# mstebelev/wormhole

Hardware: AMD Instinct MI355X
Metric: examples/sec, DiFacto FM on Criteo-1TB-shaped sparse at 1/2/4/8 MI355X (higher is better)
Workload: dtype fp32; 1 GPU; model=difacto-fm-dim64, global_batch=100000, seq_len=39, parallelism=dp1+kvshard1, minibatch_per_gpu=100000, threshold=100, nnz_per_example=39

## Files before the change

### csrc/bind/fm_ops.cc

```cpp
#include "kv_store.h"
#include "localize_ahead.h"
#include "ps_ops.h"
#include "step_rt.h"
#include "store_guard.h"

#include <c10/hip/HIPCachingAllocator.h>
#include <c10/hip/HIPGuard.h>

#include <cmath>
#include <cstring>
#include <memory>

#include "host/linear_guard_plan.h"

namespace wh_bind {
namespace {

void check_vstride(int64_t vstride) {
  TORCH_CHECK(vstride == 0 || (vstride >= 4 && vstride <= 256 && (vstride & (vstride - 1)) == 0),
              "vstride must be 0 or 4 * 2^k <= 256, got ", vstride);
}

int loss_flags(int64_t loss, const Tensor& met) {
  return (int)loss | (met.numel() >= 5 ? 256 : 0);
// ... 554 lines not shown
      const bool fuse_now = fused_v_ && vc.data_ptr() == store_->V_.data_ptr();
      auto bw = fm_backward_impl(csc_off, csc_row, csc_val, fw[1], fw[2], hdr, vc, vs_,
                                 fuse_now ? &fuse : nullptr, planned ? &bwd : nullptr);
      if (post_on_)
        fm_grad_post(bw[1], m, dim_, clip_, dropout_, seed_ + 7919 * step + 1, gnorm_);
      ht.mark(4);
      auc_acc_side(fw[0], label, auc_sum);
      ht.mark(6);
      store_->difacto_push_after(slot, hdr, bw[0], bw[1], hp_, threshold_, l1_shrk_, seed_,
                                 fuse_now ? c10::optional<Tensor>(ucnt) : c10::nullopt);
      ht.mark(5);
    } else if (train) {
      auc_acc_side(fw[0], label, auc_sum);
    }
    return py::make_tuple(fw[0], U, m);
  }

  void reset() { ahead_.reset(); }
  bool direct() const { return direct_; }
  bool fused_v() const { return fused_v_; }
  int64_t grows() const { return guard_.grows(); }
  int64_t vgrows() const { return guard_.vgrows(); }
  std::vector<int64_t> guard_sync() {
    if (guard_.stale()) guard_.after();
    return guard_.sync();
  }

 private:
  KVStore* store_;
  std::vector<double> hp_;
  int64_t threshold_;
  bool l1_shrk_;
  int64_t seed_, loss_;
  int vs_ = 0;
  double clip_ = 0, dropout_ = 0;
  bool gnorm_ = false, post_on_ = false, direct_ = false, fused_v_ = false;
  int64_t dim_ = 0;
  StoreGuard guard_;
  LocalizeAhead ahead_;
  std::unique_ptr<HostSplit> timing_{host_split("difacto native step")};
};

}

void bind_fm(py::module_& m) {
  py::class_<LinearStep>(m, "LinearStep")
      .def(py::init<KVStore*, int64_t, double, double, double, double, int64_t, double, bool>(),
           py::arg("store"), py::arg("algo"), py::arg("alpha"), py::arg("beta"), py::arg("l1"),
           py::arg("l2"), py::arg("loss"), py::arg("max_load") = 0.7, py::arg("direct") = true,
           py::keep_alive<1, 2>())
      .def("step", &LinearStep::step, py::arg("keys"), py::arg("offset"), py::arg("val"),
           py::arg("label"), py::arg("train"), py::arg("met"), py::arg("auc_sum"),
           py::arg("next_keys") = py::none(), py::arg("next_offset") = py::none(),
           py::arg("next_val") = py::none(), py::arg("ready") = 0)
      .def("reset", &LinearStep::reset)
      .def("guard_sync", &LinearStep::guard_sync)
      .def_property_readonly("grows", &LinearStep::grows)
      .def_property_readonly("direct", [](const LinearStep& l) { return l.direct(); })
      .def_property("pushes", &LinearStep::pushes, &LinearStep::set_pushes);
  py::class_<DifactoStep>(m, "DifactoStep")
      .def(py::init<KVStore*, std::vector<double>, int64_t, bool, int64_t, int64_t,
                    std::vector<double>, double, bool, bool>(),
           py::arg("store"), py::arg("hp"), py::arg("threshold"), py::arg("l1_shrk"),
           py::arg("seed"), py::arg("loss"), py::arg("post"), py::arg("max_load"),
           py::arg("direct"), py::arg("fused_v") = true, py::keep_alive<1, 2>())
      .def("step", &DifactoStep::step, py::arg("keys"), py::arg("offset"), py::arg("val"),
           py::arg("label"), py::arg("train"), py::arg("data_pass"), py::arg("met"),
           py::arg("auc_sum"), py::arg("step"), py::arg("next_keys") = py::none(),
           py::arg("next_offset") = py::none(), py::arg("next_val") = py::none(),
           py::arg("ready") = 0)
      .def("reset", &DifactoStep::reset)
      .def("guard_sync", &DifactoStep::guard_sync)
      .def_property_readonly("direct", &DifactoStep::direct)
      .def_property_readonly("fused_v", &DifactoStep::fused_v)
      .def_property_readonly("grows", &DifactoStep::grows)
      .def_property_readonly("vgrows", &DifactoStep::vgrows);
  m.def("fm_forward", &fm_forward);
  m.def("set_cu_reserve", [](int64_t n) { wh::fm_set_cu_reserve((int)n); },
        "CUs the persistent FM kernels leave free for concurrent collectives");
  m.def("cu_reserve", []() { return (int64_t)wh::fm_cu_reserve(); });
  m.def("set_fm_bwd_pack", [](bool on) { wh::fm_set_bwd_pack(on); },
        "FM backward: pack small single-chunk keys, one lane group per key (default on)");
  m.def("fm_bwd_pack", []() { return wh::fm_bwd_pack(); });
  m.def("fm_backward", &fm_backward);
  m.def("fm_backward_plan", &fm_backward_plan, py::arg("csc_off"), py::arg("csc_row"),
        py::arg("hdr"), py::arg("vc_rows"), py::arg("nrows"), py::arg("vstride"),
        py::arg("two_pass") = false);
  m.def("fm_backward_run", &fm_backward_run);
  m.def("difacto_open_pull_plan", &difacto_open_pull_plan, py::arg("store"), py::arg("keys"),
        py::arg("insert"), py::arg("cnt"), py::arg("h"), py::arg("threshold"),
        py::arg("l1_shrk"), py::arg("seed"), py::arg("direct"), py::arg("csc_off"),
        py::arg("csc_row"), py::arg("nrows"),
        "(tests) the open with the backward's chunk plan: (slot, hdr, vc, vpos, plan)");
  m.def("fm_backward_plan_totals", &fm_backward_plan_totals, py::arg("plan"),
        py::arg("csc_off"), py::arg("nnz"), py::arg("vstride"),
        "(tests) a backward plan's chunk totals {scalar, V}");
  m.def("fm_grad_post", &fm_grad_post);
  m.def("vstride_for", &vstride_for);
  m.def("spmv_t", &spmv_t, py::arg("csc_off"), py::arg("csc_row"), py::arg("csc_val"),
        py::arg("p"));
}

}
```

### csrc/hip/fm.hip

```cpp
#include "wh_common.h"
#include <string>
#include "kv_device.h"
#include "wh_chunk_plan.h"
#include "wh_kernels.h"
#include "wh_lookback.h"
#include "wh_loss.h"

#include <algorithm>
#include <cstdlib>
#include <type_traits>

namespace wh {
namespace {

constexpr int kThreads = 256;
constexpr int kFwdBlocks = 2048;

template <int G>
struct Shape {
  static constexpr int SUB = 64 / G;
  static constexpr int NI = G;
#ifndef WH_FM_TI
#define WH_FM_TI 4
#endif
  static constexpr int TI = G < WH_FM_TI ? G : WH_FM_TI;
  static constexpr int VS = 4 * G;
};

__device__ float kZeroRow[256];

template <int G>
__device__ __forceinline__ void stage_pairs(int2* st, int lane, int idx_val, float f) {
  using S = Shape<G>;
  st[(lane % S::SUB) * S::NI + lane / S::SUB] = make_int2(idx_val, __float_as_int(f));
  __builtin_amdgcn_fence(__ATOMIC_RELEASE, "wavefront");
  __builtin_amdgcn_wave_barrier();
  __builtin_amdgcn_fence(__ATOMIC_ACQUIRE, "wavefront");
}

template <int G>
__device__ __forceinline__ int stage_pairs_compact(int2* st, int lane, int vid, float f) {
  using S = Shape<G>;
  const bool has = vid >= 0;
  const uint64_t m = __ballot(has);
  const int nv = __popcll(m);
  const int pos = __popcll(m & ((1ull << lane) - 1ull));
  if (has) st[(pos % S::SUB) * S::NI + pos / S::SUB] = make_int2(vid, __float_as_int(f));
  __builtin_amdgcn_fence(__ATOMIC_RELEASE, "wavefront");
  __builtin_amdgcn_wave_barrier();
  __builtin_amdgcn_fence(__ATOMIC_ACQUIRE, "wavefront");
  return nv;
}

template <int G>
__global__ __launch_bounds__(kThreads) void k_fm_fwd(int64_t nrows, const int64_t* __restrict__ off,
                                                     const int32_t* __restrict__ lid,
                                                     const float* __restrict__ val,
                                                     const float2* __restrict__ hdr,
                                                     const float* __restrict__ vc, int vstride,
                                                     const float* __restrict__ label, int loss,
                                                     float* __restrict__ py_out,
                                                     float* __restrict__ dual_out,
                                                     float* __restrict__ xv, double* part,
                                                     double* met, unsigned int* ticket, int acc5) {
  using S = Shape<G>;
  __shared__ double sh[kThreads / 64];
  __shared__ int2 stage[kThreads / 64][64];
  const int lane = threadIdx.x & 63, gl = lane & (G - 1), sub = lane / G;
  const int64_t nw = (int64_t)gridDim.x * (kThreads / 64);
  const int64_t w0 =
      __builtin_amdgcn_readfirstlane((int)(((int64_t)blockIdx.x * kThreads + threadIdx.x) >> 6));
  double m_objv = 0, m_objw = 0, m_corr = 0, m_n = 0;
  auto bounds = [&](int64_t r, int64_t& b, int64_t& e) {
    if (r < nrows) {
      b = off[r];
      e = off[r + 1];
    } else {
      b = e = 0;
    }
  };
  auto load_ids = [&](int64_t b, int64_t e, int& l, float& x) {
    const bool ok = b + lane < e;
    l = ok ? lid[b + lane] : -1;
    x = ok ? (val ? val[b + lane] : 1.f) : 0.f;
  };
  auto load_hdr = [&](int l) {
    return l >= 0 ? hdr[l] : make_float2(0.f, __int_as_float(-1));
  };
  int2* st = stage[threadIdx.x >> 6];
  auto gather = [&](int vid, float x, float4& s, float4& q2, bool prefetch_first,
                    auto&& prefetch) {
    const int n = stage_pairs_compact<G>(st, lane, vid, x);
#pragma unroll
    for (int t0 = 0; t0 < S::NI; t0 += S::TI) {
      if (t0 * S::SUB >= n) break;
      float4 v[S::TI];
      float xs[S::TI];
#pragma unroll
      for (int t = 0; t < S::TI; ++t) {
        const int2 e = st[sub * S::NI + t0 + t];
        const bool live = (t0 + t) * S::SUB + sub < n;
        xs[t] = live ? __int_as_float(e.y) : 0.f;
        const float* src = live ? vc + (uint32_t)e.x * (uint32_t)S::VS : kZeroRow;
        v[t] = reinterpret_cast<const float4*>(src)[gl];
      }
      if (t0 == 0 && prefetch_first) prefetch();
#pragma unroll
      for (int t = 0; t < S::TI; ++t) {
        const float xu = xs[t], xx = xu * xu;
        s.x += xu * v[t].x; s.y += xu * v[t].y; s.z += xu * v[t].z; s.w += xu * v[t].w;
        q2.x += xx * v[t].x * v[t].x; q2.y += xx * v[t].y * v[t].y;
        q2.z += xx * v[t].z * v[t].z; q2.w += xx * v[t].w * v[t].w;
      }
    }
  };
  int64_t r = w0;
  int64_t bc, ec, bn, en, b2, e2, b3 = 0, e3 = 0;
  bounds(r, bc, ec);
  bounds(r + nw, bn, en);
  bounds(r + 2 * nw, b2, e2);
  int lc, ln, l2 = -1;
  float xc, xn, x2 = 0.f;
  load_ids(bc, ec, lc, xc);
  float2 hc = load_hdr(lc), hn = make_float2(0.f, 0.f);
  load_ids(bn, en, ln, xn);
  for (; r < nrows; r += nw) {
    float4 s = make_float4(0.f, 0.f, 0.f, 0.f), q2 = s;
    float wl = xc * hc.x;
    bool fetched = false;
    auto prefetch = [&]() {
      hn = load_hdr(ln);
      load_ids(b2, e2, l2, x2);
      bounds(r + 3 * nw, b3, e3);
      fetched = true;
    };
    gather(__float_as_int(hc.y), xc, s, q2, true, prefetch);
    if (!fetched) prefetch();
    for (int64_t pb = bc + 64; pb < ec; pb += 64) {
      int l;
      float x;
      load_ids(pb, ec, l, x);
      const float2 h = load_hdr(l);
      wl += x * h.x;
      gather(__float_as_int(h.y), x, s, q2, false, prefetch);
    }
#pragma unroll
    for (int o = G; o < 64; o <<= 1) {
      s.x += __shfl_xor(s.x, o, 64); s.y += __shfl_xor(s.y, o, 64);
      s.z += __shfl_xor(s.z, o, 64); s.w += __shfl_xor(s.w, o, 64);
      q2.x += __shfl_xor(q2.x, o, 64); q2.y += __shfl_xor(q2.y, o, 64);
      q2.z += __shfl_xor(q2.z, o, 64); q2.w += __shfl_xor(q2.w, o, 64);
    }
    const float wsum = wave_sum(wl);
    float pt = (s.x * s.x - q2.x) + (s.y * s.y - q2.y) + (s.z * s.z - q2.z) + (s.w * s.w - q2.w);
    pt = group_sum<G>(pt);
    if (sub == 0) reinterpret_cast<float4*>(xv + r * vstride)[gl] = s;
    if (lane == 0) {
      const float p = wsum + 0.5f * pt;
      const float y = label[r];
      const LossOut o = eval_loss(loss, y, p);
      const LossOut ow = eval_loss(loss, y, wsum);
      py_out[r] = p;
      dual_out[r] = o.dual;
      m_objv += o.objv;
      m_objw += ow.objv;
      m_corr += ((y > 0.f && p > 0.f) || (y <= 0.f && p <= 0.f)) ? 1.0 : 0.0;
      m_n += 1.0;
    }
    bc = bn; ec = en; xc = xn; hc = hn;
    bn = b2; en = e2; ln = l2; xn = x2;
    b2 = b3; e2 = e3;
  }
  block_partials(part, sh, m_objv, m_objw, m_corr, m_n, met, ticket, acc5);
}

template <int G>
__global__ __launch_bounds__(kThreads) void k_lin_fwd(int64_t nrows, const int64_t* __restrict__ off,
                                                      const int32_t* __restrict__ lid,
                                                      const float* __restrict__ val,
                                                      const float* __restrict__ w, int wstride,
                                                      const float* __restrict__ label, int loss,
                                                      float* __restrict__ py_out,
                                                      float* __restrict__ dual_out, double* part,
                                                      double* met, unsigned int* ticket, int acc5) {
  __shared__ double sh[kThreads / 64];
  const int gl = threadIdx.x & (G - 1);
  const int64_t ngroups = (int64_t)gridDim.x * (kThreads / G);
  double m_objv = 0, m_corr = 0, m_n = 0;
  for (int64_t row = ((int64_t)blockIdx.x * kThreads + threadIdx.x) / G; row < nrows;
       row += ngroups) {
    float acc = 0.f;
    const int64_t b = off[row], e = off[row + 1];
    for (int64_t j = b + gl; j < e; j += G) {
      const int32_t l = lid[j];
      if (wstride == 1) acc += (val ? val[j] : 1.f) * w[l];
// ... 60 lines not shown
                                                         Lookback lb, int ntiles,
                                                         int64_t* off_s_tot, int64_t* off_v_tot,
                                                         ChunkOut out) {
  __shared__ uint32_t shs[16];
  __shared__ int sht;
  const int tile = lb_tile(lb, ntiles, &sht);
  const int64_t k0 = (int64_t)tile * kPlanTile + threadIdx.x * kPlanPer;
  int64_t co[kPlanPer + 1];
#pragma unroll
  for (int r = 0; r <= kPlanPer; ++r) co[r] = k0 + r <= nuniq ? csc_off[k0 + r] : 0;
  int32_t vid[kPlanPer];
#pragma unroll
  for (int r = 0; r < kPlanPer; ++r) vid[r] = k0 + r < nuniq ? key_vidx(hdr, k0 + r) : -1;
  uint32_t c[2] = {0u, 0u};
  uint32_t nc[kPlanPer];
#pragma unroll
  for (int r = 0; r < kPlanPer; ++r) {
    nc[r] = k0 + r < nuniq ? (uint32_t)key_chunks(co[r + 1] - co[r], vid[r] >= 0) : 0u;
    c[vid[r] >= 0 ? 1 : 0] += nc[r];
  }
  uint32_t ex[2], tot[2];
  lb_block_scan<2>(lb, tile, c, ex, tot, shs);
  if (tile == ntiles - 1 && threadIdx.x == 0) {
    *off_s_tot = tot[0];
    *off_v_tot = tot[1];
  }
#pragma unroll
  for (int r = 0; r < kPlanPer; ++r) {
    const int isv = vid[r] >= 0;
    emit_key(out, (int32_t)(k0 + r), isv ? ex[1] : ex[0], (int32_t)nc[r], (int32_t)co[r],
             (int32_t)(co[r + 1] - co[r]), vid[r], isv);
    ex[isv ? 1 : 0] += nc[r];
  }
}

constexpr int kBuckets = 256;
constexpr int kDigits = 2 * kBuckets;
constexpr int kBucketBlocks = 128;
constexpr int kBucketU = 8;

__device__ __forceinline__ int row_bucket(int row, int shift) {
  const int b = row >> shift;
  return b < kBuckets ? b : kBuckets - 1;
}

__device__ __forceinline__ bool small_chunk(int z, int small_n) { return z >= 1 && z <= small_n; }

template <int D>
__device__ __forceinline__ int chunk_digit(int row, int shift, int z, int small_n) {
  const int b = row_bucket(row, shift);
  return D == kBuckets ? b : b * 2 + (small_chunk(z, small_n) ? 0 : 1);
}

template <int D>
__global__ __launch_bounds__(kThreads) void k_vchunk_hist(const int64_t* __restrict__ nchunk_p,
                                                          const int4* __restrict__ meta,
                                                          const int32_t* __restrict__ csc_row,
                                                          int shift, int small_n, int32_t* hist) {
  __shared__ int32_t h[D];
  for (int i = threadIdx.x; i < D; i += kThreads) h[i] = 0;
  __syncthreads();
  const int64_t n = *nchunk_p;
  const int64_t per = (n + gridDim.x - 1) / gridDim.x;
  const int64_t c0 = per * blockIdx.x, c1 = c0 + per < n ? c0 + per : n;
  for (int64_t cb = c0 + threadIdx.x; cb < c1; cb += kThreads * kBucketU) {
    int idx[kBucketU], z[kBucketU], row[kBucketU];
#pragma unroll
    for (int u = 0; u < kBucketU; ++u) {
      const int64_t c = cb + (int64_t)u * kThreads;
      idx[u] = c < c1 ? meta[c].y : -1;
      z[u] = D != kBuckets && c < c1 ? meta[c].z : 0;
    }
#pragma unroll
    for (int u = 0; u < kBucketU; ++u) row[u] = idx[u] >= 0 ? csc_row[idx[u]] : -1;
#pragma unroll
    for (int u = 0; u < kBucketU; ++u)
      if (row[u] >= 0) atomicAdd(&h[chunk_digit<D>(row[u], shift, z[u], small_n)], 1);
  }
  __syncthreads();
  for (int i = threadIdx.x; i < D; i += kThreads) hist[blockIdx.x * D + i] = h[i];
}

constexpr int kScanThreads = 1024;

template <int D>
__global__ __launch_bounds__(kScanThreads) void k_vchunk_scan(int32_t* hist) {
  constexpr int kParts = kScanThreads / D, kPer = kBucketBlocks / kParts;
  constexpr int kKeep = kPer <= 32 ? kPer : 32;
  __shared__ int32_t part[kParts][D];
  __shared__ int32_t excl[D];
  __shared__ int32_t wtot[D / 64];
  const int b = threadIdx.x & (D - 1), q = threadIdx.x / D;
  int32_t v[kKeep];
  int32_t sum = 0;
#pragma unroll
  for (int i0 = 0; i0 < kPer; i0 += kKeep) {
#pragma unroll
    for (int i = 0; i < kKeep; ++i) v[i] = hist[(q * kPer + i0 + i) * D + b];
#pragma unroll
    for (int i = 0; i < kKeep; ++i) sum += v[i];
  }
  part[q][b] = sum;
  __syncthreads();
  if (q == 0) {
    int32_t t = 0;
#pragma unroll
    for (int r = 0; r < kParts; ++r) t += part[r][b];
    const int lane = b & 63;
    int32_t x = t;
#pragma unroll
    for (int o = 1; o < 64; o <<= 1) {
      const int32_t y = __shfl_up(x, o, 64);
      if (lane >= o) x += y;
    }
    if (lane == 63) wtot[b >> 6] = x;
    excl[b] = x - t;
  }
  __syncthreads();
  int32_t base = excl[b];
  for (int w = 0; w < (b >> 6); ++w) base += wtot[w];
  for (int r = 0; r < q; ++r) base += part[r][b];
#pragma unroll
  for (int i0 = 0; i0 < kPer; i0 += kKeep) {
    if (kPer > kKeep) {
#pragma unroll
      for (int i = 0; i < kKeep; ++i) v[i] = hist[(q * kPer + i0 + i) * D + b];
    }
#pragma unroll
    for (int i = 0; i < kKeep; ++i) {
      hist[(q * kPer + i0 + i) * D + b] = base;
      base += v[i];
    }
  }
}

template <int D>
__global__ __launch_bounds__(kThreads) void k_vchunk_scatter(const int64_t* __restrict__ nchunk_p,
                                                             const int4* __restrict__ meta,
                                                             const int32_t* __restrict__ csc_row,
                                                             int shift, int small_n,
                                                             const int32_t* __restrict__ hist,
                                                             int4* out) {
  __shared__ int32_t base[D];
  for (int i = threadIdx.x; i < D; i += kThreads) base[i] = hist[blockIdx.x * D + i];
  __syncthreads();
  const int64_t n = *nchunk_p;
  const int64_t per = (n + gridDim.x - 1) / gridDim.x;
  const int64_t c0 = per * blockIdx.x, c1 = c0 + per < n ? c0 + per : n;
  for (int64_t cb = c0 + threadIdx.x; cb < c1; cb += kThreads * kBucketU) {
    int4 m[kBucketU];
    int row[kBucketU];
#pragma unroll
    for (int u = 0; u < kBucketU; ++u) {
      const int64_t c = cb + (int64_t)u * kThreads;
      m[u] = c < c1 ? meta[c] : make_int4(0, -1, 0, 0);
    }
#pragma unroll
    for (int u = 0; u < kBucketU; ++u) row[u] = m[u].y >= 0 ? csc_row[m[u].y] : -1;
#pragma unroll
    for (int u = 0; u < kBucketU; ++u)
      if (row[u] >= 0)
        out[atomicAdd(&base[chunk_digit<D>(row[u], shift, m[u].z, small_n)], 1)] = m[u];
  }
}

__global__ __launch_bounds__(kThreads) void k_bwd_scalar(const int64_t* __restrict__ nchunk_p,
                                                         const int32_t* __restrict__ chunk_key,
                                                         const int32_t* __restrict__ chunk_beg,
                                                         const int64_t* __restrict__ csc_off,
                                                         const int32_t* __restrict__ csc_row,
                                                         const float* __restrict__ csc_val,
                                                         const float* __restrict__ dual,
                                                         float* __restrict__ gw_out,
                                                         float* __restrict__ part_gw) {
  const int64_t c = (int64_t)blockIdx.x * kThreads + threadIdx.x;
  if (c >= *nchunk_p) return;
  const int k = chunk_key[c];
  const int kb = (int)csc_off[k], ke = (int)csc_off[k + 1];
  const int b = chunk_beg[c];
  const int e = b + kChunkS < ke ? b + kChunkS : ke;
  float gw = 0.f;
  int p = b;
  for (; p + 3 < e; p += 4) {
    int i[4];
    float x[4];
#pragma unroll
    for (int u = 0; u < 4; ++u) {
      i[u] = csc_row[p + u];
      x[u] = csc_val ? csc_val[p + u] : 1.f;
    }
#pragma unroll
    for (int u = 0; u < 4; ++u) gw += dual[i[u]] * x[u];
  }
  for (; p < e; ++p) gw += dual[csc_row[p]] * (csc_val ? csc_val[p] : 1.f);
  if (ke - kb <= kChunkS) gw_out[k] = gw;
  else if (part_gw) part_gw[c] = gw;
  else atomicAdd(gw_out + k, gw);
}

template <int G, bool FUSED>
__global__ __launch_bounds__(kThreads) void k_bwd_v(const int64_t* __restrict__ nchunk_p,
                                                    const int4* __restrict__ meta,
                                                    const int32_t* __restrict__ csc_row,
                                                    const float* __restrict__ csc_val,
                                                    const float* __restrict__ dual,
                                                    const float* __restrict__ xv,
                                                    const float* __restrict__ vc, int vstride,
                                                    float* __restrict__ gw_out,
                                                    float* __restrict__ gvc,
                                                    float* __restrict__ part_gw,
                                                    float* __restrict__ part_gv, float* fv,
                                                    float* fvg, DifactoHP hp, int pack) {
  using S = Shape<G>;
  constexpr bool kSplit = 64 / G >= 4;
  const float* vrows = FUSED ? fv : vc;
  __shared__ int2 stage[kThreads / 64][64];
  int2* st = stage[threadIdx.x >> 6];
  const int lane = threadIdx.x & 63, gl = lane & (G - 1), sub = lane / G;
  const int64_t nch = *nchunk_p, nw = (int64_t)gridDim.x * (kThreads / 64);
  const bool can_pack = pack != 0 && S::SUB > 1;
  const int gs = can_pack ? S::SUB : 1;
  const int64_t ngrp = (nch + gs - 1) / gs;
  const int wv = __builtin_amdgcn_readfirstlane((int)(threadIdx.x >> 6));
  const int64_t w0 = (gridDim.x & 7) == 0
                         ? (int64_t)(blockIdx.x & 7) * (nw / 8) + (blockIdx.x >> 3) * (kThreads / 64) + wv
                         : (int64_t)blockIdx.x * (kThreads / 64) + wv;
  const int4 kNone = make_int4(0, 0, 0, -1);
  const int64_t e_last = nch > 0 ? nch - 1 : 0;
// ... 242 lines not shown
  if ((m.z >> 8) == 0 || (int64_t)m.y != csc_off[m.x]) return;
  const int64_t cnt = csc_off[m.x + 1] - m.y;
  const int64_t n = (cnt + kChunkV - 1) / kChunkV;
  float g = 0.f;
  for (int64_t q = 0; q < n; ++q) g += part_gw[c + q];
  for (int d = lane; d < vstride; d += 64) {
    float a = 0.f;
    for (int64_t q = 0; q < n; ++q) a += part_gv[(c + q) * vstride + d];
    gvc[(int64_t)m.w * vstride + d] = a;
  }
  if (lane == 0) gw_out[m.x] = g;
}

__global__ __launch_bounds__(kThreads) void k_grad_post(const int64_t* __restrict__ m_p,
                                                        float* gvc, int vstride, int dim,
                                                        float clip, float dropout, uint64_t seed,
                                                        double* sumsq) {
  __shared__ double sh[kThreads / 64];
  const int64_t total = *m_p * vstride;
  double ss = 0;
  for (int64_t t = (int64_t)blockIdx.x * kThreads + threadIdx.x; t < total;
       t += (int64_t)gridDim.x * kThreads) {
    const int64_t r = t / vstride;
    const int d = (int)(t % vstride);
    if (d >= dim) continue;
    float v = gvc[t];
    if (clip > 0.f) v = fminf(fmaxf(v, -clip), clip);
    if (dropout > 0.f && uhash01(seed, (uint64_t)r, (uint64_t)d) > 1.f - dropout) v = 0.f;
    gvc[t] = v;
    ss += (double)v * v;
  }
  if (sumsq) {
    const double s = block_sum_d(ss, sh);
    if (threadIdx.x == 0) atomicAdd(sumsq, s);
  }
}

__global__ __launch_bounds__(kThreads) void k_grad_scale(const int64_t* __restrict__ m_p,
                                                         float* gvc, int vstride, int dim,
                                                         const double* sumsq) {
  const int64_t t = (int64_t)blockIdx.x * kThreads + threadIdx.x;
  const double n2 = *sumsq;
  if (n2 < 1e-10 || t / vstride >= *m_p || (int)(t % vstride) >= dim) return;
  gvc[t] = (float)(gvc[t] / sqrt(n2));
}

}

template <typename F>
static void dispatch_g(int G, F&& f) {
  switch (G) {
    case 1: f(std::integral_constant<int, 1>()); break;
    case 2: f(std::integral_constant<int, 2>()); break;
    case 4: f(std::integral_constant<int, 4>()); break;
    case 8: f(std::integral_constant<int, 8>()); break;
    case 16: f(std::integral_constant<int, 16>()); break;
    case 32: f(std::integral_constant<int, 32>()); break;
    case 64: f(std::integral_constant<int, 64>()); break;
    default:
      fprintf(stderr, "fm.hip: no kernel for vstride %d (4 * 2^k <= 256 only)\n", 4 * G);
      abort();
  }
}

int64_t fm_fwd_partials() { return 4 * kFwdBlocks; }
int64_t fwd_ticket_words() { return kArriveWords; }

static int g_cu_reserve = 0;

void fm_set_cu_reserve(int cus) { g_cu_reserve = cus < 0 ? 0 : cus; }
int fm_cu_reserve() { return g_cu_reserve; }

static int g_bwd_pack = -1;

void fm_set_bwd_pack(bool on) { g_bwd_pack = on ? 1 : 0; }
bool fm_bwd_pack() {
  if (g_bwd_pack < 0) {
    const char* e = std::getenv("WH_FM_BWD_PACK");
    g_bwd_pack = !(e && std::string(e) == "0");
  }
  return g_bwd_pack == 1;
}

static int device_cus() {
  static int cus = 0;
  if (cus == 0) {
    int dev = 0;
    WH_HIP_CHECK(hipGetDevice(&dev));
    WH_HIP_CHECK(hipDeviceGetAttribute(&cus, hipDeviceAttributeMultiprocessorCount, dev));
  }
  return std::max(1, cus - std::min(g_cu_reserve, cus / 2));
}

template <typename K>
static int resident_blocks(K kernel, int cap) {
  const int cus = device_cus();
  int per_cu = 0;
  WH_HIP_CHECK(hipOccupancyMaxActiveBlocksPerMultiprocessor(&per_cu, kernel, kThreads, 0));
  const int n = std::max(1, per_cu) * cus;
  return n < cap ? n : cap;
}

void fm_forward(int64_t nrows, const int64_t* offset, const int32_t* lid, const float* val,
                const float* w_or_hdr, const float* vc, int vstride, const float* label, int loss,
                float* py, float* dual, float* xv, double* met, double* part,
                unsigned int* ticket, hipStream_t s) {
  if (nrows <= 0) return;
  const int acc5 = (loss >> 8) & 1;
  loss &= 0xff;
  if (vstride == 0) {
    constexpr int G = 8;
    const int nblk = grid_for(nrows * G, kThreads, kFwdBlocks);
    hipLaunchKernelGGL(k_lin_fwd<G>, dim3(nblk), dim3(kThreads), 0, s, nrows, offset, lid, val,
                       w_or_hdr, 1, label, loss, py, dual, part, met, ticket, acc5);
    return;
  }
  const float2* hdr = reinterpret_cast<const float2*>(w_or_hdr);
  dispatch_g(vstride / 4, [&](auto g) {
    constexpr int G = decltype(g)::value;
    const int nblk =
        grid_for(nrows * 64, kThreads, resident_blocks(k_fm_fwd<G>, kFwdBlocks));
    hipLaunchKernelGGL(k_fm_fwd<G>, dim3(nblk), dim3(kThreads), 0, s, nrows, offset, lid, val,
                       hdr, vc, vstride, label, loss, py, dual, xv, part, met, ticket, acc5);
  });
}

void lin_forward_strided(int64_t nrows, const int64_t* offset, const int32_t* lid,
                         const float* val, const float* w, int wstride, const float* label,
                         int loss, float* py, float* dual, double* met, double* part,
                         unsigned int* ticket, hipStream_t s) {
  if (nrows <= 0) return;
  const int acc5 = (loss >> 8) & 1;
  loss &= 0xff;
  constexpr int G = 8;
  const int nblk = grid_for(nrows * G, kThreads, kFwdBlocks);
  hipLaunchKernelGGL(k_lin_fwd<G>, dim3(nblk), dim3(kThreads), 0, s, nrows, offset, lid, val, w,
                     wstride, label, loss, py, dual, part, met, ticket, acc5);
}

static int64_t scalar_cap(int64_t nuniq, int64_t nnz) { return nuniq + nnz / kChunkS + 1; }
static int64_t v_cap(int64_t nuniq, int64_t nnz) { return nuniq + nnz / kChunkV + 1; }

static int bucket_shift(int64_t nrows) {
  int shift = 0;
  while ((((nrows - 1) >> shift) >= kBuckets)) ++shift;
  return shift;
}

int64_t fm_bwd_layout(int64_t nuniq, int64_t nnz, int vstride, bool deterministic,
                      FmBwdLayout* out) {
  int64_t at = 0;
  auto carve = [&](int64_t bytes) {
    const int64_t o = at;
    at += (bytes + 255) / 256 * 256;
    return o;
  };
  const int64_t cap_s = scalar_cap(nuniq, nnz), cap_v = vstride > 0 ? v_cap(nuniq, nnz) : 0;
  FmBwdLayout l;
  l.key_s = carve(cap_s * 4);
  l.beg_s = carve(cap_s * 4);
  l.meta_v = carve(2 * cap_v * 16);
  l.hist = carve(vstride > 0 ? (int64_t)kDigits * kBucketBlocks * 4 : 0);
  l.det_s = carve(deterministic ? cap_s * 4 : 0);
  l.det_vw = carve(deterministic ? cap_v * 4 : 0);
  l.det_v = carve(deterministic ? cap_v * vstride * 4 : 0);
  l.off = carve(2 * (nuniq + 1) * 8);
  l.cnt = carve(2 * nuniq * 8);
  l.scan_tmp = carve(scan_tmp_elems(nuniq) * 8);
  if (out) *out = l;
  return at;
}

FmBwdPlanDst fm_bwd_plan_dst(const FmBwdProblem& p, void* scratch) {
  FmBwdLayout l;
  fm_bwd_layout(p.nuniq, p.nnz, p.vstride, p.deterministic, &l);
  char* base = static_cast<char*>(scratch);
  int64_t* off_s = reinterpret_cast<int64_t*>(base + l.off);
  return {p.csc_off, reinterpret_cast<int32_t*>(base + l.key_s),
          reinterpret_cast<int32_t*>(base + l.beg_s), base + l.meta_v, p.gw, p.gvc, p.vstride,
          off_s + p.nuniq, off_s + p.nuniq + 1 + p.nuniq};
}

void fm_backward(const FmBwdProblem& p, void* scratch, const Lookback* lb, hipStream_t s,
                 FmBwdPhase phase) {
  const int64_t nuniq = p.nuniq;
  if (nuniq <= 0) return;
  const int vstride = p.vstride;
  const float2* hdr = vstride > 0 ? reinterpret_cast<const float2*>(p.hdr) : nullptr;
  FmBwdLayout l;
  fm_bwd_layout(nuniq, p.nnz, vstride, p.deterministic, &l);
  char* base = static_cast<char*>(scratch);
  int32_t* key_s = reinterpret_cast<int32_t*>(base + l.key_s);
  int32_t* beg_s = reinterpret_cast<int32_t*>(base + l.beg_s);
  int4* meta_v = reinterpret_cast<int4*>(base + l.meta_v);
  int64_t* off_s = reinterpret_cast<int64_t*>(base + l.off);
  int64_t* off_v = off_s + nuniq + 1;
  const int64_t cap_s = scalar_cap(nuniq, p.nnz), cap_v = v_cap(nuniq, p.nnz);
  const bool bucket =
      hdr && !p.deterministic && p.nrows * (int64_t)vstride * 4 > ((int64_t)2 << 20);
  int4* meta_sorted = bucket ? meta_v + cap_v : meta_v;
  const bool pack = fm_bwd_pack();
  if (phase == FmBwdPhase::kAll || phase == FmBwdPhase::kPlan) {
    const ChunkOut out = {key_s, beg_s, meta_v, p.gw, p.gvc, vstride};
    const int64_t ntiles = (nuniq + kPlanTile - 1) / kPlanTile;
    if (lb && ntiles <= kLbMaxTiles) {
      hipLaunchKernelGGL(k_chunk_plan, dim3((unsigned)ntiles), dim3(kThreads), 0, s, nuniq,
                         p.csc_off, hdr, *lb, (int)ntiles, off_s + nuniq, off_v + nuniq, out);
    } else {
      int64_t* cnt_s = reinterpret_cast<int64_t*>(base + l.cnt);
      int64_t* cnt_v = cnt_s + nuniq;
      int64_t* scan_tmp = reinterpret_cast<int64_t*>(base + l.scan_tmp);
      const dim3 grid(grid_for(nuniq, kThreads));
      hipLaunchKernelGGL(k_chunk_count, grid, dim3(kThreads), 0, s, nuniq, p.csc_off, hdr, cnt_s,
                         cnt_v);
      scan_i64(cnt_s, off_s, nuniq, scan_tmp, s);
      if (hdr) scan_i64(cnt_v, off_v, nuniq, scan_tmp, s);
      hipLaunchKernelGGL(k_chunk_fill, grid, dim3(kThreads), 0, s, nuniq, p.csc_off, off_s, off_v,
                         hdr, out);
    }
  }
  if (phase != FmBwdPhase::kRun && bucket) {
    int32_t* hist = reinterpret_cast<int32_t*>(base + l.hist);
    const int shift = bucket_shift(std::max<int64_t>(p.nrows, 1));
    const int G = vstride / 4;
    const int small_n = pack && G < 64 ? std::min(G, WH_FM_TI) : 0;
    auto sort = [&](auto d) {
      constexpr int D = decltype(d)::value;
      hipLaunchKernelGGL(k_vchunk_hist<D>, dim3(kBucketBlocks), dim3(kThreads), 0, s,
                         off_v + nuniq, meta_v, p.csc_row, shift, small_n, hist);
      hipLaunchKernelGGL(k_vchunk_scan<D>, dim3(1), dim3(kScanThreads), 0, s, hist);
      hipLaunchKernelGGL(k_vchunk_scatter<D>, dim3(kBucketBlocks), dim3(kThreads), 0, s,
                         off_v + nuniq, meta_v, p.csc_row, shift, small_n, hist, meta_sorted);
    };
    if (small_n > 0) sort(std::integral_constant<int, kDigits>());
    else sort(std::integral_constant<int, kBuckets>());
  }
  if (phase == FmBwdPhase::kPlan || phase == FmBwdPhase::kBucket) return;
  const bool det = p.deterministic;
  float* pgs = det ? reinterpret_cast<float*>(base + l.det_s) : nullptr;
  float* pgv_w = det ? reinterpret_cast<float*>(base + l.det_vw) : nullptr;
  float* pgv = det ? reinterpret_cast<float*>(base + l.det_v) : nullptr;
  hipLaunchKernelGGL(k_bwd_scalar, dim3(grid_for(cap_s, kThreads)), dim3(kThreads), 0, s,
                     off_s + nuniq, key_s, beg_s, p.csc_off, p.csc_row, p.csc_val, p.dual, p.gw,
                     pgs);
  if (det)
    hipLaunchKernelGGL(k_bwd_reduce_s, dim3(grid_for(cap_s, kThreads)), dim3(kThreads), 0, s,
                       off_s + nuniq, key_s, beg_s, p.csc_off, pgs, p.gw);
  if (!hdr) return;
  dispatch_g(vstride / 4, [&](auto g) {
    constexpr int G = decltype(g)::value;
    auto run = [&](auto kernel, const float* vc) {
      const int64_t vblk = std::min<int64_t>((cap_v + 3) / 4, resident_blocks(kernel, 2048));
      hipLaunchKernelGGL(kernel, dim3((unsigned)vblk), dim3(kThreads), 0, s, off_v + nuniq,
                         meta_sorted, p.csc_row, p.csc_val, p.dual, p.xv, vc, vstride, p.gw,
                         p.gvc, pgv_w, pgv, p.fuse_v, p.fuse_vg, p.fuse_hp, pack ? 1 : 0);
    };
    if (p.fuse_v && p.fuse_v != p.vc) {
      fprintf(stderr, "fm.hip: the fused update needs vc to be the V slab itself\n");
      abort();
    }
    if (p.fuse_v) run(k_bwd_v<G, true>, nullptr);
    else run(k_bwd_v<G, false>, p.vc);
  });
  if (det)
    hipLaunchKernelGGL(k_bwd_reduce_v, dim3(grid_for(cap_v * 64, kThreads)), dim3(kThreads), 0, s,
                       off_v + nuniq, meta_v, p.csc_off, pgv_w, pgv, vstride, p.gw, p.gvc);
}

void fm_grad_post(const int64_t* m, int64_t m_cap, float* gvc, int vstride, int dim, float clip,
                  float dropout, uint64_t seed, double* sumsq, hipStream_t s) {
  if (m_cap <= 0 || vstride == 0) return;
  hipLaunchKernelGGL(k_grad_post, dim3(grid_for(m_cap * vstride, kThreads, 1024)), dim3(kThreads),
                     0, s, m, gvc, vstride, dim, clip, dropout, seed, sumsq);
}

void fm_grad_scale(const int64_t* m, int64_t m_cap, float* gvc, int vstride, int dim,
                   const double* sumsq, hipStream_t s) {
  if (m_cap <= 0 || vstride == 0) return;
  hipLaunchKernelGGL(k_grad_scale, dim3(grid_for(m_cap * vstride, kThreads)), dim3(kThreads), 0,
                     s, m, gvc, vstride, dim, sumsq);
}

}
```

### csrc/hip/wh_kernels.h

```cpp
#pragma once
#include <hip/hip_runtime.h>
#include <stdint.h>

namespace wh {

int64_t scan_tmp_elems(int64_t n);
void scan_i32(const int32_t* in, int64_t* out, int64_t n, int64_t* tmp, hipStream_t s);
void scan_i64(const int64_t* in, int64_t* out, int64_t n, int64_t* tmp, hipStream_t s);
constexpr int kLbMaxTiles = 1 << 16;
constexpr int kLbChannels = 3;
struct Lookback {
  unsigned long long* gran;
  unsigned int* ticket;
  unsigned int* err;
  unsigned int epoch;
};
int64_t lookback_ws_words();
Lookback lookback_bind(void* ws);

void loc_insert(const uint64_t* keys, int64_t nnz, uint64_t* tkeys, int64_t tsize,
                int32_t* slot_of, int64_t* overflow, hipStream_t s);
void key_mod(uint64_t* keys, int64_t n, uint64_t m, hipStream_t s);
int64_t loc_owner_blocks(int64_t tsize);
void loc_owner_count(const uint64_t* tkeys, int64_t tsize, int nshard, int64_t* blkcnt,
// ... 80 lines not shown
  int algo;
  float alpha, beta, l1, l2;
  float sgd_eta;
};
void linear_pull(const KVTable& t, const int32_t* slot, int64_t n, float* out, hipStream_t s);
void linear_push(const KVTable& t, const int32_t* slot, const float* grad, int64_t n,
                 LinearHP hp, hipStream_t s);

struct DifactoHP {
  float alpha, beta, l1, l2;
  float v_alpha, v_beta, v_l2;
  float v_init;
  uint32_t threshold;
  int l1_shrk;
  uint64_t seed;
};
void difacto_push_cnt(const KVTable& t, const int32_t* slot, const float* cnt,
                      const int32_t* cnti, int64_t n, DifactoHP hp, hipStream_t s);
void difacto_pull_hdr(const KVTable& t, const int32_t* slot, int64_t n, int l1_shrk, float* hdr,
                      int32_t* vflag, hipStream_t s);
void difacto_pull_rows(const KVTable& t, const int32_t* slot, int64_t n, const int32_t* vflag,
                       const int64_t* vpos, float* hdr, float* vc, hipStream_t s);
void difacto_push(const KVTable& t, const int32_t* slot, const float* hdr, const float* gw,
                  const float* gvc, int64_t n, DifactoHP hp, hipStream_t s,
                  const int32_t* ucnt = nullptr);
void vidx_renumber(float* hdr, int64_t n, int32_t* flag_tmp, int64_t* pos_tmp, int64_t* scan_tmp,
                   hipStream_t s);
bool difacto_pull_fused(const KVTable& t, const int32_t* slot, int64_t n, int l1_shrk,
                        const Lookback& lb, float* hdr, int64_t* vpos, float* vc, hipStream_t s);
struct FmBwdPlanDst;
bool difacto_open_pull(const KVTable& t, const uint64_t* keys, int64_t n, const int32_t* cnt,
                       DifactoHP hp, int insert, const Lookback& lb, int32_t* slot, float* hdr,
                       int64_t* vpos, float* vc, hipStream_t s,
                       const FmBwdPlanDst* plan = nullptr);
bool vidx_renumber_fused(float* hdr, int64_t n, const Lookback& lb, int64_t* count,
                         hipStream_t s);

struct PsPrep {
  uint32_t* chain = nullptr;
  int64_t n = 0;
  int32_t* vbase = nullptr;
};
bool ps_open(const KVTable& t, const uint64_t* keys, const int32_t* rec, int64_t n, int use_cnt,
             DifactoHP hp, int insert, int chains, uint32_t epoch, int32_t* vbase,
             const int64_t* segS, const int64_t* segHS, int P, const Lookback& lb, int32_t* slot,
             float* w_out, int64_t* vpos, uint32_t* chain, uint8_t* head, float* rbuf,
             int64_t* vcnt, hipStream_t s, int prepped = 0);
bool ps_push(const KVTable& t, const int32_t* slot, const int64_t* vpos, const uint32_t* chain,
             const uint8_t* head, int64_t n, const int64_t* segS, const int64_t* segHS, int P,
             const float* gbuf, DifactoHP hp, hipStream_t s, PsPrep prep = PsPrep());
void ps_records(const uint64_t* uniq, const int32_t* ucnt, int64_t U, int32_t* rec,
                hipStream_t s);
bool ps_c0(const int64_t* owner_cnt, const int64_t* vcnt, int S, int P, int64_t flag,
           int64_t* send, int64_t* payload, hipStream_t s, int loop = 0);
bool ps_push_linear(const KVTable& t, const int32_t* slot, const uint32_t* chain,
                    const uint8_t* head, int64_t n, const int64_t* segS, int P, const float* g,
                    LinearHP hp, double t0, hipStream_t s, PsPrep prep = PsPrep());
bool ps_unpack(const float* rbuf, int64_t U, int vstride, const int64_t* segS,
               const int64_t* segHS, const int64_t* vrecv, int P, float* hdr, int64_t* rows_total,
               hipStream_t s);
bool ps_pack_gw(const float* gw, int64_t U, int vstride, const int64_t* segS,
                const int64_t* segHS, const int64_t* vrecv, int P, float* gbuf, hipStream_t s);

int64_t fm_fwd_partials();
int64_t fwd_ticket_words();
void lin_forward_strided(int64_t nrows, const int64_t* offset, const int32_t* lid,
                         const float* val, const float* w, int wstride, const float* label,
                         int loss, float* py, float* dual, double* met, double* part,
                         unsigned int* ticket, hipStream_t s);
int ld_rows_per_tile(int64_t nnz, int64_t nrows);
int ld_tile_table(int64_t nnz);
void ld_touch(const KVTable& t, const uint64_t* keys, const int64_t* off, int64_t nrows,
              int64_t nnz, int R, uint32_t stamp, int insert, int32_t* lid, int32_t* tlist,
              unsigned int* tcnt, int32_t* ovf, unsigned int* ovf_cnt, hipStream_t s);
void ld_backward(const int32_t* lid, const float* val, const int64_t* off, int64_t nrows,
                 int64_t nnz, int R, const float* dual, float* grad, hipStream_t s);
void ld_push(const KVTable& t, int64_t ntiles, int T, const int32_t* tlist,
             const unsigned int* tcnt, const int32_t* ovf, unsigned int* ovf_cnt, float* grad,
             LinearHP hp, hipStream_t s);
void fm_set_cu_reserve(int cus);
int fm_cu_reserve();
void fm_set_bwd_pack(bool on);
bool fm_bwd_pack();
void fm_forward(int64_t nrows, const int64_t* offset, const int32_t* lid, const float* val,
                const float* w_or_hdr, const float* vc, int vstride, const float* label, int loss,
                float* py, float* dual, float* xv, double* met, double* part,
                unsigned int* ticket, hipStream_t s);
struct FmBwdProblem {
  int64_t nuniq, nnz, nrows;
  const int64_t* csc_off;
  const int32_t* csc_row;
  const float* csc_val;
  const float *dual, *xv;
  const float *hdr, *vc;
  int vstride;
  float *gw, *gvc;
  bool deterministic;
  float* fuse_v = nullptr;
  float* fuse_vg = nullptr;
  DifactoHP fuse_hp = {};
};
constexpr int kChunkV = 64;
enum class FmBwdPhase { kAll, kPlan, kRun, kBucket, kBucketRun };
struct FmBwdLayout {
  int64_t key_s, beg_s;
  int64_t meta_v;
  int64_t hist;
  int64_t det_s, det_vw, det_v;
  int64_t off;
  int64_t cnt, scan_tmp;
};
int64_t fm_bwd_layout(int64_t nuniq, int64_t nnz, int vstride, bool deterministic,
                      FmBwdLayout* out = nullptr);
struct FmBwdPlanDst {
  const int64_t* csc_off;
  int32_t *key_s, *beg_s;
  void* meta_v;
  float *gw, *gvc;
  int vstride;
  int64_t *tot_s, *tot_v;
};
FmBwdPlanDst fm_bwd_plan_dst(const FmBwdProblem& p, void* scratch);
void fm_backward(const FmBwdProblem& p, void* scratch, const Lookback* lb, hipStream_t s,
                 FmBwdPhase phase);
void fm_grad_post(const int64_t* m, int64_t m_cap, float* gvc, int vstride, int dim, float clip,
                  float dropout, uint64_t seed, double* sumsq, hipStream_t s);
void fm_grad_scale(const int64_t* m, int64_t m_cap, float* gvc, int vstride, int dim,
                   const double* sumsq, hipStream_t s);

void spmv(int64_t nrows, const int64_t* off, const int32_t* col, const float* val, const float* x,
          float* y, hipStream_t s);
size_t auc_sort_tmp_bytes(int64_t n);
void sort_by_score(const float* py, const float* label, int64_t n, float* py_sorted,
                   float* label_sorted, void* tmp, size_t tmp_bytes, hipStream_t s);
void auc_from_sorted(const float* label_sorted, int64_t n, double* out, int64_t* tmp_i64,
                     hipStream_t s);
int64_t auc_ws_bytes(int64_t n);
int64_t auc_ws_persistent_bytes();
int64_t auc_ws_lohi_offset();
void auc_accumulate(const float* py, const float* label, int64_t n, void* persist, void* scratch,
                    double* auc_sum, hipStream_t s);

void synth_criteo(int64_t nrows, uint64_t seed, uint64_t step, const int64_t* card,
                  int nfield, uint64_t* keys, float* label, int64_t* offset, hipStream_t s);

int kmeans_ks(int f);
bool kmeans_x3_supported(int f);
int64_t kmeans_x3_xp_bytes(int64_t n, int f);
int64_t kmeans_x3_cp_bytes(int k, int f);
void kmeans_pack_x3(const float* X, int64_t n, int f, void* Xp3, hipStream_t s);
void kmeans_pack_c3(const float* C, int k, int f, void* Cp3, hipStream_t s);
void kmeans_assign_x3(const void* Xp3, const float* xnorm, const float* X, int64_t n, int f,
                      const void* Cp3, const float* C, int k, int32_t* assign, float* score,
                      int32_t* amb, float* ct, hipStream_t s);
void kmeans_pack_x(const float* X, int64_t n, int f, float* Xp, hipStream_t s);
int64_t kmeans_cp_elems(int k, int f);
void kmeans_pack_c(const float* C, int k, int f, float* Cp, hipStream_t s);
void kmeans_assign(const float* Xp, int64_t n, int f, const float* Cp, int k, int32_t* assign,
                   float* score, hipStream_t s);
void kmeans_accum(const float* X, int64_t n, int f, const int32_t* assign, float* sums,
                  hipStream_t s);
int64_t kmeans_accum_scratch(int64_t n, int k);
void kmeans_assign_csr(const int64_t* off, const int32_t* col, const float* val, int64_t n,
                       const float* Ct, int K, int Kp, int32_t* assign, hipStream_t s);
void kmeans_accum_csr(const int64_t* off, const int32_t* col, const float* val, int64_t n,
                      const int32_t* assign, int F, float* sums, hipStream_t s);
// ... 221 lines not shown
```

Measured before the change: 159.2 million examples/s.

## Parallelize backward bucket-sort scan across blocks and restructure forward gather batching

The backward radix-style bucket scan moves from a single 1024-thread block to 16 blocks, each owning a slice of digits. Cross-digit prefix bases are now computed inside the scatter kernel from a new per-digit totals array, which removes a serial single-block step. The forward gather now uses a templated batch depth, optional via env var or setter, and loads dead lanes from the row-0 address instead of a zero row, masking them during accumulation. Default depth stays 4, so the forward change mostly alters masking and load addressing, while the scan parallelization always runs.

```diff
diff --git a/csrc/bind/fm_ops.cc b/csrc/bind/fm_ops.cc
--- a/csrc/bind/fm_ops.cc
+++ b/csrc/bind/fm_ops.cc
@@ -660,6 +660,9 @@
   m.def("set_fm_bwd_pack", [](bool on) { wh::fm_set_bwd_pack(on); },
         "FM backward: pack small single-chunk keys, one lane group per key (default on)");
   m.def("fm_bwd_pack", []() { return wh::fm_bwd_pack(); });
+  m.def("set_fm_fwd_depth", [](int64_t d) { wh::fm_set_fwd_depth((int)d); },
+        "FM forward: 10 = a headline row's gathers in one batch; anything else = batches of 4 (default)");
+  m.def("fm_fwd_depth", []() { return (int64_t)wh::fm_fwd_depth(); });
   m.def("fm_backward", &fm_backward);
   m.def("fm_backward_plan", &fm_backward_plan, py::arg("csc_off"), py::arg("csc_row"),
         py::arg("hdr"), py::arg("vc_rows"), py::arg("nrows"), py::arg("vstride"),
diff --git a/csrc/hip/fm.hip b/csrc/hip/fm.hip
--- a/csrc/hip/fm.hip
+++ b/csrc/hip/fm.hip
@@ -25,6 +25,11 @@
 #endif
   static constexpr int TI = G < WH_FM_TI ? G : WH_FM_TI;
   static constexpr int VS = 4 * G;
+};
+
+template <int G>
+struct FwdDepth {
+  static constexpr int kDeep = G == 16 ? 10 : Shape<G>::TI;
 };
 
 __device__ float kZeroRow[256];
@@ -52,7 +57,7 @@
   return nv;
 }
 
-template <int G>
+template <int G, int FI>
 __global__ __launch_bounds__(kThreads) void k_fm_fwd(int64_t nrows, const int64_t* __restrict__ off,
                                                      const int32_t* __restrict__ lid,
                                                      const float* __restrict__ val,
@@ -91,26 +96,32 @@
   auto gather = [&](int vid, float x, float4& s, float4& q2, bool prefetch_first,
                     auto&& prefetch) {
     const int n = stage_pairs_compact<G>(st, lane, vid, x);
-#pragma unroll
-    for (int t0 = 0; t0 < S::NI; t0 += S::TI) {
+    if (n == 0) return;
+    const uint32_t row0 = (uint32_t)st[0].x;
+#pragma unroll
+    for (int b = 0; b < (S::NI + FI - 1) / FI; ++b) {
+      const int t0 = b * FI;
       if (t0 * S::SUB >= n) break;
-      float4 v[S::TI];
-      float xs[S::TI];
-#pragma unroll
-      for (int t = 0; t < S::TI; ++t) {
-        const int2 e = st[sub * S::NI + t0 + t];
+      float4 v[FI];
+#pragma unroll
+      for (int t = 0; t < FI; ++t) {
+        if (t0 + t >= S::NI) continue;
         const bool live = (t0 + t) * S::SUB + sub < n;
-        xs[t] = live ? __int_as_float(e.y) : 0.f;
-        const float* src = live ? vc + (uint32_t)e.x * (uint32_t)S::VS : kZeroRow;
-        v[t] = reinterpret_cast<const float4*>(src)[gl];
+        const uint32_t row = live ? (uint32_t)st[sub * S::NI + t0 + t].x : row0;
+        v[t] = reinterpret_cast<const float4*>(vc + row * (uint32_t)S::VS)[gl];
       }
       if (t0 == 0 && prefetch_first) prefetch();
-#pragma unroll
-      for (int t = 0; t < S::TI; ++t) {
-        const float xu = xs[t], xx = xu * xu;
-        s.x += xu * v[t].x; s.y += xu * v[t].y; s.z += xu * v[t].z; s.w += xu * v[t].w;
-        q2.x += xx * v[t].x * v[t].x; q2.y += xx * v[t].y * v[t].y;
-        q2.z += xx * v[t].z * v[t].z; q2.w += xx * v[t].w * v[t].w;
+      asm volatile("" ::: "memory");
+#pragma unroll
+      for (int t = 0; t < FI; ++t) {
+        if (t0 + t >= S::NI) continue;
+        const bool live = (t0 + t) * S::SUB + sub < n;
+        const float xu = live ? __int_as_float(st[sub * S::NI + t0 + t].y) : 0.f;
+        const float xx = xu * xu;
+        const float4 u = live ? v[t] : make_float4(0.f, 0.f, 0.f, 0.f);
+        s.x += xu * u.x; s.y += xu * u.y; s.z += xu * u.z; s.w += xu * u.w;
+        q2.x += xx * u.x * u.x; q2.y += xx * u.y * u.y;
+        q2.z += xx * u.z * u.z; q2.w += xx * u.w * u.w;
       }
     }
   };
@@ -337,56 +348,77 @@
 }
 
 constexpr int kScanThreads = 1024;
+constexpr int kScanBlocks = 16;
 
 template <int D>
-__global__ __launch_bounds__(kScanThreads) void k_vchunk_scan(int32_t* hist) {
-  constexpr int kParts = kScanThreads / D, kPer = kBucketBlocks / kParts;
-  constexpr int kKeep = kPer <= 32 ? kPer : 32;
-  __shared__ int32_t part[kParts][D];
-  __shared__ int32_t excl[D];
-  __shared__ int32_t wtot[D / 64];
-  const int b = threadIdx.x & (D - 1), q = threadIdx.x / D;
-  int32_t v[kKeep];
+__global__ __launch_bounds__(kScanThreads) void k_vchunk_scan(int32_t* hist, int32_t* tot) {
+  constexpr int kOwn = D / kScanBlocks;
+  constexpr int kParts = kScanThreads / kOwn;
+  constexpr int kPer = kBucketBlocks / kParts;
+  static_assert(kParts <= 64 && kPer * kParts == kBucketBlocks, "one wave scans a digit");
+  __shared__ int32_t part[kParts][kOwn + 1];
+  const int dl = threadIdx.x % kOwn, q = threadIdx.x / kOwn;
+  const int d = blockIdx.x * kOwn + dl;
+  int32_t v[kPer];
   int32_t sum = 0;
 #pragma unroll
-  for (int i0 = 0; i0 < kPer; i0 += kKeep) {
-#pragma unroll
-    for (int i = 0; i < kKeep; ++i) v[i] = hist[(q * kPer + i0 + i) * D + b];
-#pragma unroll
-    for (int i = 0; i < kKeep; ++i) sum += v[i];
-  }
-  part[q][b] = sum;
+  for (int i = 0; i < kPer; ++i) v[i] = hist[(q * kPer + i) * D + d];
+#pragma unroll
+  for (int i = 0; i < kPer; ++i) sum += v[i];
+  part[q][dl] = sum;
   __syncthreads();
-  if (q == 0) {
-    int32_t t = 0;
-#pragma unroll
-    for (int r = 0; r < kParts; ++r) t += part[r][b];
-    const int lane = b & 63;
+  {
+    const int tq = threadIdx.x % kParts, td = threadIdx.x / kParts;
+    const int32_t t = part[tq][td];
     int32_t x = t;
 #pragma unroll
-    for (int o = 1; o < 64; o <<= 1) {
-      const int32_t y = __shfl_up(x, o, 64);
-      if (lane >= o) x += y;
-    }
-    if (lane == 63) wtot[b >> 6] = x;
-    excl[b] = x - t;
+    for (int o = 1; o < kParts; o <<= 1) {
+      const int32_t y = __shfl_up(x, o, kParts);
+      if (tq >= o) x += y;
+    }
+    part[tq][td] = x - t;
+    if (tq == kParts - 1) tot[blockIdx.x * kOwn + td] = x;
   }
   __syncthreads();
-  int32_t base = excl[b];
-  for (int w = 0; w < (b >> 6); ++w) base += wtot[w];
-  for (int r = 0; r < q; ++r) base += part[r][b];
-#pragma unroll
-  for (int i0 = 0; i0 < kPer; i0 += kKeep) {
-    if (kPer > kKeep) {
-#pragma unroll
-      for (int i = 0; i < kKeep; ++i) v[i] = hist[(q * kPer + i0 + i) * D + b];
-    }
-#pragma unroll
-    for (int i = 0; i < kKeep; ++i) {
-      hist[(q * kPer + i0 + i) * D + b] = base;
-      base += v[i];
-    }
-  }
+  int32_t base = part[q][dl];
+#pragma unroll
+  for (int i = 0; i < kPer; ++i) {
+    hist[(q * kPer + i) * D + d] = base;
+    base += v[i];
+  }
+}
+
+template <int D>
+__device__ __forceinline__ void digit_bases(const int32_t* __restrict__ tot,
+                                            const int32_t* __restrict__ within, int32_t* base,
+                                            int32_t* wsum) {
+  constexpr int kPer = D / kThreads;
+  static_assert(kPer * kThreads == D, "digits split evenly over the block");
+  const int lane = threadIdx.x & 63, wave = threadIdx.x >> 6;
+  int32_t t[kPer], w[kPer];
+  int32_t sum = 0;
+#pragma unroll
+  for (int j = 0; j < kPer; ++j) {
+    t[j] = tot[threadIdx.x * kPer + j];
+    w[j] = within[threadIdx.x * kPer + j];
+    sum += t[j];
+  }
+  int32_t x = sum;
+#pragma unroll
+  for (int o = 1; o < 64; o <<= 1) {
+    const int32_t y = __shfl_up(x, o, 64);
+    if (lane >= o) x += y;
+  }
+  if (lane == 63) wsum[wave] = x;
+  __syncthreads();
+  int32_t off = x - sum;
+  for (int k = 0; k < wave; ++k) off += wsum[k];
+#pragma unroll
+  for (int j = 0; j < kPer; ++j) {
+    base[threadIdx.x * kPer + j] = off + w[j];
+    off += t[j];
+  }
+  __syncthreads();
 }
 
 template <int D>
@@ -395,10 +427,11 @@
                                                              const int32_t* __restrict__ csc_row,
                                                              int shift, int small_n,
                                                              const int32_t* __restrict__ hist,
+                                                             const int32_t* __restrict__ tot,
                                                              int4* out) {
   __shared__ int32_t base[D];
-  for (int i = threadIdx.x; i < D; i += kThreads) base[i] = hist[blockIdx.x * D + i];
-  __syncthreads();
+  __shared__ int32_t wsum[kThreads / 64];
+  digit_bases<D>(tot, hist + blockIdx.x * D, base, wsum);
   const int64_t n = *nchunk_p;
   const int64_t per = (n + gridDim.x - 1) / gridDim.x;
   const int64_t c0 = per * blockIdx.x, c1 = c0 + per < n ? c0 + per : n;
@@ -807,6 +840,17 @@
   return g_bwd_pack == 1;
 }
 
+static int g_fwd_depth = -1;
+
+void fm_set_fwd_depth(int depth) { g_fwd_depth = depth == 10 ? 10 : 4; }
+int fm_fwd_depth() {
+  if (g_fwd_depth < 0) {
+    const char* e = std::getenv("WH_FM_FWD_DEPTH");
+    g_fwd_depth = e && std::string(e) == "10" ? 10 : 4;
+  }
+  return g_fwd_depth;
+}
+
 static int device_cus() {
   static int cus = 0;
   if (cus == 0) {
@@ -843,10 +887,14 @@
   const float2* hdr = reinterpret_cast<const float2*>(w_or_hdr);
   dispatch_g(vstride / 4, [&](auto g) {
     constexpr int G = decltype(g)::value;
-    const int nblk =
-        grid_for(nrows * 64, kThreads, resident_blocks(k_fm_fwd<G>, kFwdBlocks));
-    hipLaunchKernelGGL(k_fm_fwd<G>, dim3(nblk), dim3(kThreads), 0, s, nrows, offset, lid, val,
-                       hdr, vc, vstride, label, loss, py, dual, xv, part, met, ticket, acc5);
+    const int nblk = grid_for(nrows * 64, kThreads,
+                              resident_blocks(k_fm_fwd<G, FwdDepth<G>::kDeep>, kFwdBlocks));
+    auto run = [&](auto kernel) {
+      hipLaunchKernelGGL(kernel, dim3(nblk), dim3(kThreads), 0, s, nrows, offset, lid, val, hdr,
+                         vc, vstride, label, loss, py, dual, xv, part, met, ticket, acc5);
+    };
+    if (fm_fwd_depth() == 10) run(k_fm_fwd<G, FwdDepth<G>::kDeep>);
+    else run(k_fm_fwd<G, Shape<G>::TI>);
   });
 }
 
@@ -885,7 +933,7 @@
   l.key_s = carve(cap_s * 4);
   l.beg_s = carve(cap_s * 4);
   l.meta_v = carve(2 * cap_v * 16);
-  l.hist = carve(vstride > 0 ? (int64_t)kDigits * kBucketBlocks * 4 : 0);
+  l.hist = carve(vstride > 0 ? (int64_t)kDigits * (kBucketBlocks + 1) * 4 : 0);
   l.det_s = carve(deterministic ? cap_s * 4 : 0);
   l.det_vw = carve(deterministic ? cap_v * 4 : 0);
   l.det_v = carve(deterministic ? cap_v * vstride * 4 : 0);
@@ -946,6 +994,7 @@
   }
   if (phase != FmBwdPhase::kRun && bucket) {
     int32_t* hist = reinterpret_cast<int32_t*>(base + l.hist);
+    int32_t* tot = hist + kDigits * kBucketBlocks;
     const int shift = bucket_shift(std::max<int64_t>(p.nrows, 1));
     const int G = vstride / 4;
     const int small_n = pack && G < 64 ? std::min(G, WH_FM_TI) : 0;
@@ -953,9 +1002,11 @@
       constexpr int D = decltype(d)::value;
       hipLaunchKernelGGL(k_vchunk_hist<D>, dim3(kBucketBlocks), dim3(kThreads), 0, s,
                          off_v + nuniq, meta_v, p.csc_row, shift, small_n, hist);
-      hipLaunchKernelGGL(k_vchunk_scan<D>, dim3(1), dim3(kScanThreads), 0, s, hist);
+      hipLaunchKernelGGL(k_vchunk_scan<D>, dim3(kScanBlocks), dim3(kScanThreads), 0, s, hist,
+                         tot);
       hipLaunchKernelGGL(k_vchunk_scatter<D>, dim3(kBucketBlocks), dim3(kThreads), 0, s,
-                         off_v + nuniq, meta_v, p.csc_row, shift, small_n, hist, meta_sorted);
+                         off_v + nuniq, meta_v, p.csc_row, shift, small_n, hist, tot,
+                         meta_sorted);
     };
     if (small_n > 0) sort(std::integral_constant<int, kDigits>());
     else sort(std::integral_constant<int, kBuckets>());
diff --git a/csrc/hip/wh_kernels.h b/csrc/hip/wh_kernels.h
--- a/csrc/hip/wh_kernels.h
+++ b/csrc/hip/wh_kernels.h
@@ -186,6 +186,8 @@
 int fm_cu_reserve();
 void fm_set_bwd_pack(bool on);
 bool fm_bwd_pack();
+void fm_set_fwd_depth(int depth);
+int fm_fwd_depth();
 void fm_forward(int64_t nrows, const int64_t* offset, const int32_t* lid, const float* val,
                 const float* w_or_hdr, const float* vc, int vstride, const float* label, int loss,
                 float* py, float* dual, float* xv, double* met, double* part,
```

New measurement: 169.1 million examples/s (median of 6 runs). 6.3% higher.
